# jyoung3131/oncilla

Measured on AMD Instinct MI355X. Metric: remote put/get GiB/s + p50 ocm_alloc latency, 4 KiB-1 GiB, 1/2/4/8 MI355X, higher is better.
Workload: dtype uint8

## Files before the change

### csrc/src/kernels/xfer.hip

```cpp
#include <hip/hip_runtime.h>

#include <cstring>

#include "ocm/xfer.h"
#include "xfer_copy.h"
#include "xfer_host.h"

namespace ocm {

namespace {

constexpr int kWaveSlice = (1 << kTileShift) / kWaves;
constexpr int kChunksPerWave = kWaveSlice / 1024;

template <class Cfg, bool MASKED = false>
__device__ __forceinline__ void copy_tiles(const XferArgs &a, uint32_t ext_mask = 0) {
    const uint64_t first = xfer_first_tile(a.rem_off, a.tile_shift);
    const uint64_t ntiles = xfer_tile_count(a.rem_off, a.len, a.tile_shift);
    const uint64_t r0 = a.rem_off;
    for (uint64_t ti = blockIdx.x; ti < ntiles; ti += gridDim.x) {
        if (MASKED && a.n_ext > 1) {
            const uint64_t lo = first + (ti << a.tile_shift);
            const uint64_t ts = lo > r0 ? lo : r0;
            const uint32_t e = (uint32_t)(ts >> a.unit_shift) % a.n_ext;
            if (!((ext_mask >> e) & 1u)) continue;
        }
        TileSpan s = tile_span(a, ti, first);
        copy_span<Cfg>(s.dst, s.src, s.n);
    }
}

template <int ST>
__global__ __launch_bounds__(kThreads) void xfer_reg_kernel(XferArgs a, XferDone d) {
    copy_tiles<BlockCopy<ST>>(a);
    xfer_publish(d);
}

typedef __attribute__((address_space(3))) void lds_void;
typedef const __attribute__((address_space(1))) void glob_void;

__device__ __forceinline__ bool full_aligned(const TileSpan &s) {
    return s.n == (1ull << kTileShift) && (((uintptr_t)s.dst | (uintptr_t)s.src) & 15u) == 0;
}

__device__ __forceinline__ void stage_tile(const char *src, char *buf, int wave, int lane) {
    const char *g = src + (size_t)wave * kWaveSlice + (size_t)lane * 16;
    char *l = buf + (size_t)wave * kWaveSlice;
#pragma unroll
    for (int c = 0; c < kChunksPerWave; c++)
        __builtin_amdgcn_global_load_lds((glob_void *)(g + c * 1024), (lds_void *)(l + c * 1024), 16, 0, 0);
}

template <bool NT>
__device__ __forceinline__ void drain_tile(char *dst, const char *buf, int wave, int lane) {
    const char *l = buf + (size_t)wave * kWaveSlice + (size_t)lane * 16;
    char *g = dst + (size_t)wave * kWaveSlice + (size_t)lane * 16;
    u32x4 v[kChunksPerWave];
#pragma unroll
    for (int c = 0; c < kChunksPerWave; c++) v[c] = *reinterpret_cast<const u32x4 *>(l + c * 1024);
#pragma unroll
    for (int c = 0; c < kChunksPerWave; c++)
        store16<NT>(reinterpret_cast<u32x4 *>(g + c * 1024), v[c]);
}

template <bool NT>
__device__ __forceinline__ void lds_stream(const XferArgs &a, char *lds, int wave, int lane, uint64_t ti,
                                           uint64_t first, uint64_t ntiles) {
    TileSpan cur = tile_span(a, ti, first);
    bool cur_staged = full_aligned(cur);
    if (cur_staged) stage_tile(cur.src, lds, wave, lane);
    int slot = 0;
    for (;;) {
        const uint64_t nt = ti + gridDim.x;
        TileSpan nxt;
        bool nxt_staged = false;
        if (nt < ntiles) {
            nxt = tile_span(a, nt, first);
            nxt_staged = full_aligned(nxt);
            if (nxt_staged) stage_tile(nxt.src, lds + (slot ^ 1) * (1 << kTileShift), wave, lane);
        }
        if (cur_staged) {
            if (nxt_staged)
                asm volatile("s_waitcnt vmcnt(8)" ::: "memory");
            else
                asm volatile("s_waitcnt vmcnt(0)" ::: "memory");
            drain_tile<NT>(cur.dst, lds + slot * (1 << kTileShift), wave, lane);
        } else {
            copy_span<BlockCopy<NT ? ST_NT : ST_PLAIN>>(cur.dst, cur.src, cur.n);
        }
        if (nt >= ntiles) break;
        ti = nt;
        cur = nxt;
        cur_staged = nxt_staged;
        slot ^= 1;
    }
}

template <bool NT>
__global__ __launch_bounds__(kThreads) void xfer_lds_kernel(XferArgs a, XferDone d) {
    __shared__ __attribute__((aligned(16))) char lds[2 * (1 << kTileShift)];
    const int wave = threadIdx.x >> 6, lane = threadIdx.x & 63;
    const uint64_t first = xfer_first_tile(a.rem_off, a.tile_shift);
    const uint64_t ntiles = xfer_tile_count(a.rem_off, a.len, a.tile_shift);
    uint64_t ti = blockIdx.x;
    if (ti < ntiles) lds_stream<NT>(a, lds, wave, lane, ti, first, ntiles);
    xfer_publish(d);
}

constexpr int kPcieUnroll = 2;
constexpr uint32_t kPcieTileShift = 13;
constexpr unsigned kPcieBlocksDefault = 128;

template <int SA>
using PcieCopy = CopyCfg<kThreads, kPcieUnroll, BufferAccess<kAuxNT, SA>>;

template <int SA>
__global__ __launch_bounds__(kThreads) void xfer_pcie_kernel(XferArgs a, XferDone d) {
    copy_tiles<PcieCopy<SA>>(a);
    xfer_publish(d);
}

__global__ __launch_bounds__(kThreads) void xfer_push_kernel(XferArgs a, uint32_t mask) {
    copy_tiles<BlockCopy<ST_NT>, true>(a, mask);
}

}

XferTuning xfer_tuning_from_env() {
    XferTuning t;
    const char *v = std::getenv("OCM_XFER_VARIANT");
    if (v && (!std::strcmp(v, "lds") || !std::strcmp(v, "2"))) t.variant = XFER_LDS;
    if (v && (!std::strcmp(v, "reg") || !std::strcmp(v, "1"))) t.variant = XFER_REG;
    if (v && (!std::strcmp(v, "pcie") || !std::strcmp(v, "4"))) t.variant = XFER_PCIE;
    if (v && (!std::strcmp(v, "push") || !std::strcmp(v, "5"))) t.variant = XFER_PUSH;
    t.max_blocks = kernels::env_int("OCM_XFER_BLOCKS", 0);
    t.nontemporal = kernels::env_int("OCM_XFER_NT", 1) != 0;
    t.write_through = kernels::env_int("OCM_XFER_NT", 1) == 2;
    return t;
}

hipError_t xfer_normalize(XferArgs &a) {
    if (a.n_ext < 1 || a.n_ext > (uint32_t)kXferMaxExtents) return hipErrorInvalidValue;
    a.tile_shift = kTileShift;
    if (a.n_ext > 1) {
        if (a.unit_shift < 4) return hipErrorInvalidValue;
        if (a.unit_shift < kTileShift) a.tile_shift = a.unit_shift;
    }
    return hipSuccess;
}

hipError_t xfer_launch(const XferArgs &in, const XferTuning &t, hipStream_t stream, const XferDone *done) {
    if (in.len == 0) return hipSuccess;
    XferArgs a = in;
    if (xfer_normalize(a) != hipSuccess) return hipErrorInvalidValue;
    const uint64_t ntiles = xfer_tile_count(a.rem_off, a.len, a.tile_shift);
    int variant = t.variant;
    if (variant == XFER_AUTO) variant = XFER_REG;
    const XferDone d0 = done ? *done : XferDone{};
    if (variant == XFER_PCIE) {
        if (a.tile_shift > kPcieTileShift) a.tile_shift = kPcieTileShift;
        const uint64_t tiles = xfer_tile_count(a.rem_off, a.len, a.tile_shift);
        const uint64_t cap = t.max_blocks > 0 ? (uint64_t)t.max_blocks : (uint64_t)kPcieBlocksDefault;
        const unsigned g = (unsigned)(tiles < cap ? tiles : cap);
        if (a.put && t.nontemporal)
            hipLaunchKernelGGL(xfer_pcie_kernel<kAuxSC1>, dim3(g), dim3(kThreads), 0, stream, a, d0);
        else
            hipLaunchKernelGGL(xfer_pcie_kernel<0>, dim3(g), dim3(kThreads), 0, stream, a, d0);
        return hipGetLastError();
    }
    if (a.tile_shift != kTileShift) variant = XFER_REG;
    int cap = t.max_blocks > 0 ? t.max_blocks : kernels::num_cus() * (variant == XFER_LDS ? 4 : 2);
    const unsigned grid = (unsigned)(ntiles < (uint64_t)cap ? ntiles : (uint64_t)cap);
    if (variant == XFER_LDS) {
        if (t.nontemporal)
            hipLaunchKernelGGL(xfer_lds_kernel<true>, dim3(grid), dim3(kThreads), 0, stream, a, d0);
        else
            hipLaunchKernelGGL(xfer_lds_kernel<false>, dim3(grid), dim3(kThreads), 0, stream, a, d0);
    } else {
        if (t.write_through)
            hipLaunchKernelGGL(xfer_reg_kernel<ST_WT>, dim3(grid), dim3(kThreads), 0, stream, a, d0);
        else if (t.nontemporal)
            hipLaunchKernelGGL(xfer_reg_kernel<ST_NT>, dim3(grid), dim3(kThreads), 0, stream, a, d0);
        else
            hipLaunchKernelGGL(xfer_reg_kernel<ST_PLAIN>, dim3(grid), dim3(kThreads), 0, stream, a, d0);
    }
    return hipGetLastError();
}

hipError_t xfer_push_launch(const XferArgs &in, uint32_t ext_mask, int max_blocks, hipStream_t stream) {
    if (in.len == 0 || ext_mask == 0) return hipSuccess;
    XferArgs a = in;
    if (a.put || xfer_normalize(a) != hipSuccess) return hipErrorInvalidValue;
    const uint64_t tiles = xfer_tile_count(a.rem_off, a.len, a.tile_shift);
    const uint32_t mine = (uint32_t)__builtin_popcount(ext_mask & ((1u << a.n_ext) - 1));
    const uint64_t own = a.n_ext > 1 ? (tiles * mine + a.n_ext - 1) / a.n_ext : tiles;
    const uint64_t cap = max_blocks > 0 ? (uint64_t)max_blocks : (uint64_t)kernels::num_cus() * 2;
    const unsigned g = (unsigned)(own < cap ? (own ? own : 1) : cap);
    hipLaunchKernelGGL(xfer_push_kernel, dim3(g), dim3(kThreads), 0, stream, a, ext_mask);
    return hipGetLastError();
}

hipError_t xfer_copy(void *dst, const void *src, uint64_t bytes, const XferTuning &t, hipStream_t stream) {
    XferArgs a;
    std::memset(&a, 0, sizeof(a));
    a.lin = const_cast<char *>(static_cast<const char *>(src));
    a.ext[0] = static_cast<char *>(dst);
    a.rem_off = 0;
    a.len = bytes;
    a.n_ext = 1;
    a.put = 1;
    return xfer_launch(a, t, stream);
}

}
```

### csrc/src/kernels/xfer_copy.h

```cpp
#pragma once
#include <hip/hip_runtime.h>

#include "ocm/list.h"
#include "ocm/xfer.h"

namespace ocm {

namespace {

typedef unsigned int u32x4 __attribute__((ext_vector_type(4)));

constexpr int kThreads = 256;
constexpr int kUnroll = 8;
constexpr uint32_t kTileShift = 15;
constexpr int kWaves = kThreads / 64;
static_assert(kWaves == kListWaves, "the host plans lists for workgroups of kListWaves waves");

enum StoreKind : int { ST_PLAIN = 0, ST_NT = 1, ST_WT = 2 };

__device__ __forceinline__ __amdgpu_buffer_rsrc_t span_rsrc(const void *base, uint32_t bytes) {
    const uint64_t b = reinterpret_cast<uint64_t>(base);
    const uint32_t lo = __builtin_amdgcn_readfirstlane((uint32_t)b);
    const uint32_t hi = __builtin_amdgcn_readfirstlane((uint32_t)(b >> 32));
    const uint32_t n = __builtin_amdgcn_readfirstlane(bytes);
    return __builtin_amdgcn_make_buffer_rsrc(reinterpret_cast<void *>(((uint64_t)hi << 32) | lo), 0, (int)n, 0x00020000);
}

constexpr int kAuxNT = 2, kAuxSC1 = 16;

template <int ST>
constexpr int store_aux() {
    return ST == ST_WT ? kAuxSC1 : ST == ST_NT ? kAuxNT : 0;
}
template <int ST>
constexpr int load_aux() {
    return ST == ST_WT ? kAuxSC1 : kAuxNT;
}

template <bool ATOMIC>
__device__ __forceinline__ void copy_byte(char *d, const char *s) {
    if constexpr (ATOMIC)
        __hip_atomic_store(d, __hip_atomic_load(s, __ATOMIC_RELAXED, __HIP_MEMORY_SCOPE_AGENT), __ATOMIC_RELAXED,
                           __HIP_MEMORY_SCOPE_AGENT);
    else
        *d = *s;
}

__device__ __forceinline__ uint64_t span_head(const char *dst, uint64_t n) {
    const uint64_t head = (16u - ((uintptr_t)dst & 15u)) & 15u;
    return head < n ? head : n;
}

template <bool NT>
__device__ __forceinline__ void store16(u32x4 *p, u32x4 v) {
    if constexpr (NT)
        __builtin_nontemporal_store(v, p);
    else
        *p = v;
}

template <int LA, int SA>
struct BufferAccess {
    static constexpr bool kRangeChecked = true;
    using Index = uint32_t;
    __amdgpu_buffer_rsrc_t rs, rd;
    __device__ __forceinline__ BufferAccess(char *dst, const char *src, uint32_t bytes)
        : rs(span_rsrc(src, bytes)), rd(span_rsrc(dst, bytes)) {}
    __device__ __forceinline__ u32x4 load(Index i) const {
        return __builtin_amdgcn_raw_buffer_load_b128(rs, (int)(i << 4), 0, LA);
    }
    __device__ __forceinline__ void store(Index i, u32x4 v) const {
        __builtin_amdgcn_raw_buffer_store_b128(v, rd, (int)(i << 4), 0, SA);
    }
};

template <bool NT>
struct PointerAccess {
    static constexpr bool kRangeChecked = false;
    using Index = uint64_t;
    const u32x4 *s;
    u32x4 *d;
    __device__ __forceinline__ PointerAccess(char *dst, const char *src, uint64_t)
        : s(reinterpret_cast<const u32x4 *>(src)), d(reinterpret_cast<u32x4 *>(dst)) {}
    __device__ __forceinline__ u32x4 load(Index i) const { return __builtin_nontemporal_load(s + i); }
    __device__ __forceinline__ void store(Index i, u32x4 v) const { store16<NT>(d + i, v); }
};

template <int LANES, int UNROLL, class ACCESS, bool ATOMIC_BYTES = false>
struct CopyCfg {
    static_assert(LANES == kThreads || LANES == 64, "a workgroup or one wave");
    static constexpr int kLanes = LANES, kRound = LANES * UNROLL;
    static constexpr int kVecs = UNROLL;
    static constexpr bool kAtomicBytes = ATOMIC_BYTES;
    using Access = ACCESS;
    __device__ static __forceinline__ int lane() { return LANES == 64 ? (int)(threadIdx.x & 63) : (int)threadIdx.x; }
};

template <int ST>
using BlockCopy = CopyCfg<kThreads, kUnroll, BufferAccess<load_aux<ST>(), store_aux<ST>()>, ST == ST_WT>;

template <class Cfg>
__device__ __forceinline__ void load_round(const typename Cfg::Access &acc, typename Cfg::Access::Index i,
                                           u32x4 (&v)[Cfg::kVecs]) {
#pragma unroll
    for (int k = 0; k < Cfg::kVecs; k++) v[k] = acc.load(i + k * Cfg::kLanes);
}

template <class Cfg>
__device__ __forceinline__ void store_round(const typename Cfg::Access &acc, typename Cfg::Access::Index i,
                                            const u32x4 (&v)[Cfg::kVecs]) {
#pragma unroll
    for (int k = 0; k < Cfg::kVecs; k++) acc.store(i + k * Cfg::kLanes, v[k]);
}

template <class Cfg>
__device__ __forceinline__ void copy_span(char *__restrict__ dst, const char *__restrict__ src, uint64_t n) {
    using Access = typename Cfg::Access;
    using Index = typename Access::Index;
    constexpr bool AB = Cfg::kAtomicBytes;
    const int lane = Cfg::lane();
    const uint64_t head = span_head(dst, n);
    if ((uint64_t)lane < head) copy_byte<AB>(dst + lane, src + lane);
    dst += head;
    src += head;
    n -= head;
    if (((uintptr_t)src & 15u) == 0 && (!Access::kRangeChecked || n < (1ull << 31))) {
        const Index nv = (Index)(n >> 4);
        const Access acc(dst, src, nv << 4);
        if constexpr (Access::kRangeChecked) {
            for (Index base = 0; base < nv; base += Cfg::kRound) {
                u32x4 v[Cfg::kVecs];
                load_round<Cfg>(acc, base + lane, v);
                store_round<Cfg>(acc, base + lane, v);
            }
        } else {
            Index i = lane;
            for (; i + (Cfg::kRound - Cfg::kLanes) < nv; i += Cfg::kRound) {
                u32x4 v[Cfg::kVecs];
                load_round<Cfg>(acc, i, v);
                store_round<Cfg>(acc, i, v);
            }
            for (; i < nv; i += Cfg::kLanes) acc.store(i, acc.load(i));
        }
        const uint64_t done = (uint64_t)nv << 4, tail = n & 15u;
        if ((uint64_t)lane < tail) copy_byte<AB>(dst + done + lane, src + done + lane);
    } else {
        for (uint64_t i = lane; i < n; i += Cfg::kLanes) copy_byte<AB>(dst + i, src + i);
    }
}

struct TileSpan {
    char *dst;
    const char *src;
    uint64_t n;
};

template <class Cfg>
__device__ __forceinline__ void copy_span2(const TileSpan &a, const TileSpan &b) {
    using Access = typename Cfg::Access;
    static_assert(Access::kRangeChecked, "a partial round relies on the range check");
    constexpr bool AB = Cfg::kAtomicBytes;
    const bool vec = (((uintptr_t)a.src ^ (uintptr_t)a.dst) & 15u) == 0 &&
                     (((uintptr_t)b.src ^ (uintptr_t)b.dst) & 15u) == 0 &&
                     a.n <= (uint64_t)Cfg::kRound * 16 && b.n <= (uint64_t)Cfg::kRound * 16;
    if (!vec) {
        copy_span<Cfg>(a.dst, a.src, a.n);
        copy_span<Cfg>(b.dst, b.src, b.n);
        return;
    }
    const int lane = Cfg::lane();
    const uint64_t ha = span_head(a.dst, a.n), hb = span_head(b.dst, b.n);
    if ((uint64_t)lane < ha) copy_byte<AB>(a.dst + lane, a.src + lane);
    if ((uint64_t)lane < hb) copy_byte<AB>(b.dst + lane, b.src + lane);
    const uint32_t nva = (uint32_t)((a.n - ha) >> 4), nvb = (uint32_t)((b.n - hb) >> 4);
    const Access acca(a.dst + ha, a.src + ha, nva << 4), accb(b.dst + hb, b.src + hb, nvb << 4);
    u32x4 va[Cfg::kVecs], vb[Cfg::kVecs];
    load_round<Cfg>(acca, lane, va);
    load_round<Cfg>(accb, lane, vb);
    store_round<Cfg>(acca, lane, va);
    store_round<Cfg>(accb, lane, vb);
    const uint64_t ta = (a.n - ha) & 15u, tb = (b.n - hb) & 15u;
    const uint64_t oa = ha + ((uint64_t)nva << 4), ob = hb + ((uint64_t)nvb << 4);
    if ((uint64_t)lane < ta) copy_byte<AB>(a.dst + oa + lane, a.src + oa + lane);
    if ((uint64_t)lane < tb) copy_byte<AB>(b.dst + ob + lane, b.src + ob + lane);
}

template <class E>
__device__ __forceinline__ char *stripe_ptr(const E &x, uint32_t n_ext, uint32_t unit_shift, uint64_t off) {
    if (n_ext == 1) return x.ext[0] + off;
    const uint64_t unit_mask = (1ull << unit_shift) - 1;
    const uint32_t u = (uint32_t)(off >> unit_shift);
    const uint32_t e = u % n_ext;
    const uint64_t eoff = ((uint64_t)(u / n_ext) << unit_shift) | (off & unit_mask);
    return x.ext[e] + eoff;
}

template <class E>
__device__ __forceinline__ TileSpan tile_span_of(const E &x, uint32_t n_ext, uint32_t unit_shift, uint32_t tile_shift,
                                                 char *lin, uint64_t rem_off, uint64_t len, uint32_t put, uint64_t ti,
                                                 uint64_t first_tile) {
    const uint64_t tile = 1ull << tile_shift;
    const uint64_t r0 = rem_off, r1 = rem_off + len;
    const uint64_t lo = first_tile + (ti << tile_shift);
    const uint64_t ts = lo > r0 ? lo : r0;
    const uint64_t te = (lo + tile) < r1 ? (lo + tile) : r1;
    char *rp = stripe_ptr(x, n_ext, unit_shift, ts);
    char *lp = lin + (ts - r0);
    TileSpan s;
    s.dst = put ? rp : lp;
    s.src = put ? lp : rp;
    s.n = te - ts;
    return s;
}

__device__ __forceinline__ TileSpan tile_span(const XferArgs &a, uint64_t ti, uint64_t first_tile) {
    return tile_span_of(a, a.n_ext, a.unit_shift, a.tile_shift, a.lin, a.rem_off, a.len, a.put, ti, first_tile);
}

__device__ __forceinline__ uint32_t uniform32(uint32_t v) { return __builtin_amdgcn_readfirstlane(v); }
__device__ __forceinline__ uint64_t uniform64(uint64_t v) {
    return ((uint64_t)uniform32((uint32_t)(v >> 32)) << 32) | uniform32((uint32_t)v);
}

template <class Args, class Op>
__device__ __forceinline__ uint32_t list_wave_start(const Args &a, uint32_t w, const Op **ops) {
    const bool inl = a.n_ops <= (uint32_t)(sizeof(Args::inline_ops) / sizeof(Op));
    *ops = inl ? a.inline_ops : a.ops;
    return inl ? 0u : a.wave_op[w];
}

__device__ __forceinline__ void block_release_system() {
    asm volatile("s_waitcnt vmcnt(0)" ::: "memory");
    __syncthreads();
    if (threadIdx.x == 0) __threadfence_system();
}

__device__ __forceinline__ void xfer_publish(const XferDone &d) {
    if (!d.flag) return;
    block_release_system();
    if (threadIdx.x == 0) {
        const unsigned old = __hip_atomic_fetch_add(d.cnt, 1u, __ATOMIC_ACQ_REL, __HIP_MEMORY_SCOPE_AGENT);
        if (old == gridDim.x - 1) {
            __hip_atomic_store(d.cnt, 0u, __ATOMIC_RELAXED, __HIP_MEMORY_SCOPE_AGENT);
            __hip_atomic_store(d.flag, d.val, __ATOMIC_RELEASE, __HIP_MEMORY_SCOPE_SYSTEM);
        }
    }
}

}

}
```

### csrc/src/lib/transfer.cpp

```cpp
#include "internal.h"

namespace ocmlib {



void segments(const lib_alloc *a, uint64_t rem_off, uint64_t len, std::vector<Seg> &out) {
    out.clear();
    const int n = (int)a->ext.size();
    if (n == 1 || a->stripe_unit == 0) {
        out.push_back({0, rem_off, 0, len});
        return;
    }
    const uint64_t unit = a->stripe_unit;
    uint64_t pos = rem_off, done = 0;
    while (done < len) {
        const uint64_t u = pos / unit, within = pos % unit;
        const uint64_t take = std::min(unit - within, len - done);
        out.push_back({(int)(u % n), (u / n) * unit + within, done, take});
        pos += take;
        done += take;
    }
}


int wait_event(hipEvent_t ev) {
    State &s = S();
    hipError_t e = hipSuccess;
    if (s.cfg.sync_mode == 1) {
        while ((e = hipEventQuery(ev)) == hipErrorNotReady) {
        }
    } else {
        e = hipEventSynchronize(ev);
    }
    if (e != hipSuccess) OCM_FAIL(-1, "event wait: %s", hipGetErrorString(e));
    return 0;
}

int honor_dep(lib_alloc *a, hipStream_t st, bool host_wait) {
    if (!a->dep_pending) return 0;
    a->dep_pending = false;
    hipError_t e = host_wait ? hipEventSynchronize(a->dep_ev) : hipStreamWaitEvent(st, a->dep_ev, 0);
    if (e != hipSuccess) OCM_FAIL(-1, "stream dependency: %s", hipGetErrorString(e));
    return 0;
}

int wait_alloc(lib_alloc *a) {
    State &s = S();
    if (!a || !a->async_pending) return 0;
    a->async_pending = false;
    if (!a->ev) return 0;
    DeviceGuard g(s.device);
    return wait_event(a->ev);
}

hipStream_t lane_stream(lib_alloc *a) {
    State &s = S();
    if (a->lane < 0) {
        if (s.lanes.empty()) {
            DeviceGuard g(s.device);
            for (int i = 0; i < std::max(1, s.cfg.n_lanes); i++) {
                hipStream_t st = nullptr;
                if (hipStreamCreateWithFlags(&st, hipStreamNonBlocking) != hipSuccess) {
                    (void)hipGetLastError();
                    break;
                }
                s.lanes.push_back(st);
            }
        }
        if (s.lanes.empty()) return s.stream;
        if (!s.lane_flags && s.cfg.launch_flags) {
            DeviceGuard g(s.device);
            const size_t nl = s.lanes.size();
            if (hipHostMalloc(reinterpret_cast<void **>(&s.lane_flags), nl * 128,
                              hipHostMallocCoherent | hipHostMallocMapped) != hipSuccess ||
                hipMalloc(reinterpret_cast<void **>(&s.lane_cnt), nl * 128) != hipSuccess ||
                hipMemset(s.lane_cnt, 0, nl * 128) != hipSuccess) {
                (void)hipGetLastError();
                s.cfg.launch_flags = false;
            } else {
                std::memset(s.lane_flags, 0, nl * 128);
                s.lane_flag_seq.assign(nl, 0);
            }
        }
        a->lane = s.next_lane++ % (int)s.lanes.size();
    }
    if (!a->ev) {
        DeviceGuard g(s.device);
        if (hipEventCreateWithFlags(&a->ev, hipEventDisableTiming) != hipSuccess) {
            (void)hipGetLastError();
            a->ev = nullptr;
            return s.stream;
        }
    }
    return s.lanes[a->lane];
}

int sync_stream() {
    State &s = S();
    if (!s.stream) return 0;
    DeviceGuard g(s.device);
    hipError_t e = hipSuccess;
    if (s.cfg.sync_mode == 0 || !s.done) {
        e = hipStreamSynchronize(s.stream);
    } else {
        e = hipEventRecord(s.done, s.stream);
        if (e == hipSuccess && s.cfg.sync_mode == 1) {
            while ((e = hipEventQuery(s.done)) == hipErrorNotReady) {
            }
        } else if (e == hipSuccess) {
            e = hipEventSynchronize(s.done);
        }
    }
    if (e != hipSuccess) OCM_FAIL(-1, "stream sync: %s", hipGetErrorString(e));
    return 0;
}

int async_done(lib_alloc *a, hipStream_t st) {
    State &s = S();
    if (st != s.stream && a->ev) {
        const hipError_t err = hipEventRecord(a->ev, st);
        if (err != hipSuccess) OCM_FAIL(-1, "event record failed: %s", hipGetErrorString(err));
    } else if (a->ev == nullptr && sync_stream() != 0) {
        return -1;
    }
    a->async_pending = a->ev != nullptr;
    return 0;
}

int wait_done(const XferDone &d, hipEvent_t ev) {
    for (unsigned spins = 1;; spins++) {
        if ((long long)(__atomic_load_n(d.flag, __ATOMIC_ACQUIRE) - d.val) >= 0) return 0;
        if ((spins & 4095) == 0) {
            const hipError_t e = hipEventQuery(ev);
            if (e == hipSuccess) return 0;
            if (e != hipErrorNotReady) OCM_FAIL(-1, "event wait: %s", hipGetErrorString(e));
        }
    }
}


static const XferTuning &dir_tuning(bool put) {
    State &s = S();
    const XferTuning &dt = s.dir_tuning[put ? 1 : 0];
    return dt.variant != XFER_AUTO ? dt : s.tuning;
}

static int pair_args(const lib_alloc *a, bool put, char *lin, uint64_t rem_off, uint64_t len, XferArgs *x) {
    std::memset(x, 0, sizeof(*x));
    x->lin = lin;
    x->rem_off = rem_off;
    x->len = len;
    x->put = put ? 1 : 0;
    if (pair_side(a, 0, x) < 0)
        OCM_FAIL(-1, "stripe unit %llu is not a power of two", (unsigned long long)a->stripe_unit);
    return 0;
}

static bool cpu_copies(Loc lloc, const Extent &e) {
    return S().device < 0 || (lloc != LOC_DEVICE && e.r.tier != TIER_GPU);
}

static hipError_t copy_segs(const lib_alloc *a, const Seg *segs, size_t n, bool put, char *lin, Loc lloc,
                            hipStream_t st) {
    for (const Seg *g = segs; g != segs + n; g++) {
        const Extent &e = a->ext[g->ext];
        const bool cpu = cpu_copies(lloc, e);
        char *r = (cpu ? e.hptr : e.dptr) + g->ext_off, *l = lin + g->lin_off;
        if (cpu) {
            std::memcpy(put ? r : l, put ? l : r, g->len);
            continue;
        }
        const hipError_t err = hipMemcpyAsync(put ? r : l, put ? l : r, g->len, hipMemcpyDefault, st);
        if (err != hipSuccess) return err;
    }
    return hipSuccess;
}


static int xfer_net(lib_alloc *a, bool put, char *lin, Loc lloc, uint64_t rem_off, uint64_t len) {
    State &s = S();
    std::vector<Seg> segs;
    segments(a, rem_off, len, segs);
    if (wait_alloc(a) != 0) return -1;
    if (honor_dep(a, nullptr, true) != 0) return -1;
    DeviceGuard dg(s.device);
    for (auto &g : segs) {
        const Extent &e = a->ext[g.ext];
        if (e.net) {
            if (net_piece(e, put, lin + g.lin_off, lloc, g.ext_off, g.len) != 0) return -1;
            continue;
        }
        if (copy_segs(a, &g, 1, put, lin, lloc, s.stream) != hipSuccess) OCM_FAIL(-1, "transfer launch failed");
        if (!cpu_copies(lloc, e) && sync_stream() != 0) return -1;
    }
    return 0;
}

static int xfer_cpu(lib_alloc *a, bool put, char *lin, Loc lloc, uint64_t rem_off, uint64_t len) {
    std::vector<Seg> segs;
    segments(a, rem_off, len, segs);
    (void)copy_segs(a, segs.data(), segs.size(), put, lin, lloc, nullptr);
    return 0;
}

static int xfer_service(lib_alloc *a, bool put, char *lin, uint64_t rem_off, uint64_t len) {
    State &s = S();
    XferArgs x;
    if (pair_args(a, put, lin, rem_off, len, &x) != 0) return -2;
    if (wait_alloc(a) != 0) return -2;
    if (honor_dep(a, nullptr, true) != 0) return -2;
    const unsigned solo = (!put && !a->any_gpu) ? std::min(s.cfg.svc_solo_tiles, s.cfg.svc_solo_tiles_host_get)
                                                : s.cfg.svc_solo_tiles;
    return service_xfer(x, solo, a->any_gpu, a->any_peer || s.cfg.svc_force_strict);
}

static int xfer_push(lib_alloc *a, char *lin, uint64_t rem_off, uint64_t len, hipStream_t st, bool async) {
    before_launch();
    if (push_get(a, lin, rem_off, len, st, async) != 0) return -1;
    return async ? async_done(a, st) : 0;
}

static int xfer_kernel(lib_alloc *a, bool put, char *lin, uint64_t rem_off, uint64_t len, hipStream_t st, bool async,
                       XferDone *done) {
    State &s = S();
    if ((s.cfg.svc_park_kernel || !a->any_gpu) && len > s.cfg.svc_limit(a)) service_park();
    before_launch();
    XferArgs x;
    if (pair_args(a, put, lin, rem_off, len, &x) != 0) return -1;
    XferTuning t = dir_tuning(put);
    if (t.variant == XFER_AUTO) {
        bool same_gpu = true;
        for (auto &e : a->ext) same_gpu &= e.r.tier == TIER_GPU && e.r.owner_gpu == s.device;
        t.variant = !a->any_gpu ? XFER_PCIE : (same_gpu && len <= (256ull << 20)) ? XFER_LDS : XFER_REG;
    }
    XferDone dn;
    if (done && async && len <= s.cfg.launch_flag_max && s.cfg.launch_flags && s.lane_flags && st != s.stream &&
        a->lane >= 0 && a->ev) {
        dn.flag = s.lane_flags + (size_t)a->lane * 16;
        dn.cnt = s.lane_cnt + (size_t)a->lane * 32;
        dn.val = ++s.lane_flag_seq[(size_t)a->lane];
    }
    const hipError_t err = xfer_launch(x, t, st, dn.flag ? &dn : nullptr);
    if (err != hipSuccess) OCM_FAIL(-1, "transfer launch failed: %s", hipGetErrorString(err));
    if (done) *done = dn;
    return async ? async_done(a, st) : sync_stream();
}

static int xfer_dma(lib_alloc *a, bool put, char *lin, Loc lloc, uint64_t rem_off, uint64_t len, hipStream_t st,
                    bool async) {
    service_park();
    std::vector<Seg> segs;
    segments(a, rem_off, len, segs);
    bool cpu_piece = false;
    for (auto &g : segs) cpu_piece |= cpu_copies(lloc, a->ext[g.ext]);
    hipError_t err = hipSuccess;
    if (cpu_piece && (err = hipStreamSynchronize(st)) != hipSuccess)
        OCM_FAIL(-1, "ordering a host copy after queued work: %s", hipGetErrorString(err));
    err = copy_segs(a, segs.data(), segs.size(), put, lin, lloc, st);
    if (err != hipSuccess) OCM_FAIL(-1, "transfer launch failed: %s", hipGetErrorString(err));
    return async ? async_done(a, st) : sync_stream();
}

int xfer(lib_alloc *a, bool put, char *lin, Loc lloc, uint64_t rem_off, uint64_t len, bool async, XferDone *done) {
    State &s = S();
    if (done) *done = XferDone{};
    if (len == 0) return 0;
    if (a->any_net) return xfer_net(a, put, lin, lloc, rem_off, len);
    if (s.device < 0) return xfer_cpu(a, put, lin, lloc, rem_off, len);
    DeviceGuard guard(s.device);
    const bool lin_dev = lloc == LOC_DEVICE;
    const bool dma_pick = dir_tuning(put).variant == XFER_DMA;
    if (lin_dev && a->all_dev_ok && !async && len <= s.cfg.svc_limit(a) && !dma_pick) {
        const int rc = xfer_service(a, put, lin, rem_off, len);
        if (rc == 0) return 0;
        if (rc == -2) return -1;
        OCM_WARN("copy service failed (%s); falling back to launches", last_error());
        s.cfg.svc_max = 0;
    }
    if (!async && wait_alloc(a) != 0) return -1;
    hipStream_t st = async ? lane_stream(a) : s.stream;
    if (honor_dep(a, st, false) != 0) return -1;
    const bool use_kernel =
        lin_dev && !dma_pick && (a->any_gpu || s.cfg.host_engine_kernel || len <= s.cfg.host_kernel_max);
    if (!use_kernel) return xfer_dma(a, put, lin, lloc, rem_off, len, st, async);
    if (!put && a->all_gpu && dir_tuning(false).variant == XFER_PUSH) return xfer_push(a, lin, rem_off, len, st, async);
    return xfer_kernel(a, put, lin, rem_off, len, st, async, done);
}


void push_release() {
    State &s = S();
    for (auto &kv : s.push) {
        DeviceGuard g(kv.first);
        if (kv.second.stream) (void)hipStreamSynchronize(kv.second.stream);
    }
}

static PushDev *push_dev(int d) {
    State &s = S();
    PushDev &p = s.push[d];
    if (p.ready) return &p;
    DeviceGuard g(d);
    if (d != s.device) {
        int can = 0;
        if (hipDeviceCanAccessPeer(&can, d, s.device) != hipSuccess || !can)
            OCM_FAIL(nullptr, "push get: GPU %d cannot reach GPU %d", d, s.device);
        const hipError_t pe = hipDeviceEnablePeerAccess(s.device, 0);
        if (pe != hipSuccess && pe != hipErrorPeerAccessAlreadyEnabled)
            OCM_FAIL(nullptr, "push get: peer access %d -> %d: %s", d, s.device, hipGetErrorString(pe));
        (void)hipGetLastError();
    }
    if (!p.stream && hipStreamCreateWithFlags(&p.stream, hipStreamNonBlocking) != hipSuccess)
        OCM_FAIL(nullptr, "push get: no stream on GPU %d", d);
    if (!p.done && hipEventCreateWithFlags(&p.done, hipEventDisableTiming) != hipSuccess)
        OCM_FAIL(nullptr, "push get: no event on GPU %d", d);
    p.ready = true;
    return &p;
}

int push_get(lib_alloc *a, char *lin, uint64_t rem_off, uint64_t len, hipStream_t st, bool async) {
    State &s = S();
    if (!a->all_gpu || a->any_net) OCM_FAIL(-1, "push get needs every extent in a GPU's HBM");
    std::map<int, uint32_t> owners;
    for (size_t i = 0; i < a->ext.size(); i++) {
        const int d = a->ext[i].r.owner_gpu;
        if (d < 0) OCM_FAIL(-1, "push get: extent %zu has no owner GPU", i);
        owners[d] |= 1u << i;
    }
    DeviceGuard g(s.device);
    if (!s.push_order && hipEventCreateWithFlags(&s.push_order, hipEventDisableTiming) != hipSuccess)
        OCM_FAIL(-1, "push get: no event");
    if (hipEventRecord(s.push_order, st) != hipSuccess) OCM_FAIL(-1, "push get: ordering event");
    std::vector<PushDev *> used;
    for (auto &kv : owners) {
        const int d = kv.first;
        PushDev *p = push_dev(d);
        if (!p) return -1;
        XferArgs x;
        if (pair_args(a, false, lin, rem_off, len, &x) != 0) return -1;
        for (size_t i = 0; i < a->ext.size(); i++) {
            x.ext[i] = nullptr;
            if (!((kv.second >> i) & 1u)) continue;
            x.ext[i] = extent_view(a->ext[i], d);
            if (!x.ext[i]) return -1;
        }
        DeviceGuard gd(d);
        hipError_t e = hipStreamWaitEvent(p->stream, s.push_order, 0);
        if (e == hipSuccess) e = xfer_push_launch(x, kv.second, s.dir_tuning[0].max_blocks, p->stream);
        if (e == hipSuccess) e = hipEventRecord(p->done, p->stream);
        if (e != hipSuccess) OCM_FAIL(-1, "push get on GPU %d: %s", d, hipGetErrorString(e));
        used.push_back(p);
        s.push_launches++;
    }
    for (PushDev *p : used) {
        const hipError_t e = async ? hipStreamWaitEvent(st, p->done, 0) : hipEventSynchronize(p->done);
        if (e != hipSuccess) OCM_FAIL(-1, "push get completion: %s", hipGetErrorString(e));
    }
    return 0;
}

int copy_local(void *dst, Loc dl, const void *src, Loc sl, size_t n) {
    State &s = S();
    if (n == 0) return 0;
    if (dl != LOC_DEVICE && sl != LOC_DEVICE) {
        std::memcpy(dst, src, n);
        return 0;
    }
    DeviceGuard g(s.device);
    hipError_t e;
    before_launch();
    if (dl == LOC_DEVICE && sl == LOC_DEVICE) {
        XferTuning t = s.tuning;
        if (t.variant == XFER_AUTO) t.variant = n <= (256ull << 20) ? XFER_LDS : XFER_REG;
        e = xfer_copy(dst, src, n, t, s.stream);
    } else
    {
        e = hipMemcpyAsync(dst, src, n, hipMemcpyDefault, s.stream);
    }
    if (e != hipSuccess) OCM_FAIL(-1, "local copy failed: %s", hipGetErrorString(e));
    return sync_stream();
}


}
```

Measured before the change: 52.84.

## Software-pipeline register copy kernel with buffer loads and route same-GPU traffic to it

Replaces the per-tile register copy with a double-buffered pipeline that issues the next tile's buffer loads before storing the current one, using explicit vmcnt waits so loads and stores overlap. For single-extent transfers under 2 GiB it builds one buffer resource and only advances an offset per tile, avoiding per-tile span computation. Misaligned head and tail tiles are handled separately by the first and last blocks. Auto selection no longer picks the LDS-staged kernel for same-GPU transfers and always uses the register path for GPU memory, which could be worse if the LDS path was better for local copies.

```diff
diff --git a/csrc/src/kernels/xfer.hip b/csrc/src/kernels/xfer.hip
--- a/csrc/src/kernels/xfer.hip
+++ b/csrc/src/kernels/xfer.hip
@@ -30,9 +30,103 @@
     }
 }
 
+__device__ __forceinline__ bool full_tiles_aligned(const XferArgs &a) {
+    uintptr_t m = (uintptr_t)a.lin - a.rem_off;
+#pragma unroll
+    for (uint32_t e = 0; e < (uint32_t)kXferMaxExtents; e++)
+        if (e < a.n_ext) m |= (uintptr_t)a.ext[e];
+    return (m & 15u) == 0;
+}
+
+template <bool FLAT>
+__device__ __forceinline__ TileRef full_tile_ref(const XferArgs &a, const TileRef &whole, uint64_t ti, uint64_t first) {
+    if constexpr (FLAT) {
+        TileRef t = whole;
+        t.off = (uint32_t)(first + (ti << kTileShift) - a.rem_off);
+        return t;
+    } else {
+        const TileSpan s = tile_span(a, ti, first);
+        return TileRef{span_rsrc(s.src, 1u << kTileShift), span_rsrc(s.dst, 1u << kTileShift), 0u};
+    }
+}
+
+template <int ST, bool FLAT>
+__device__ __forceinline__ void pipe_tiles(const XferArgs &a, uint64_t first, uint64_t t0, uint64_t t1) {
+    static_assert(3 * kUnroll < 64, "the waits below count up to 2 * kUnroll operations");
+    const uint64_t grid = gridDim.x;
+    uint64_t ti = blockIdx.x;
+    if (ti < t0) ti += grid;
+    if (ti >= t1) return;
+    const int voff = (int)threadIdx.x * 16;
+    TileRef whole{};
+    if constexpr (FLAT) {
+        const char *rem = a.ext[0] + a.rem_off;
+        whole.rs = span_rsrc(a.put ? a.lin : rem, (uint32_t)a.len);
+        whole.rd = span_rsrc(a.put ? rem : a.lin, (uint32_t)a.len);
+    }
+    u32x4 va[kUnroll], vb[kUnroll];
+    TileRef ra = full_tile_ref<FLAT>(a, whole, ti, first), rb;
+    tile_load<ST>(ra, voff, va);
+    if ((ti += grid) >= t1) {
+        vm_retire_to<0>();
+        tile_store<ST>(ra, voff, va);
+        return;
+    }
+    rb = full_tile_ref<FLAT>(a, whole, ti, first);
+    tile_load<ST>(rb, voff, vb);
+    vm_retire_to<kUnroll>();
+    tile_store<ST>(ra, voff, va);
+    for (;;) {
+        if ((ti += grid) >= t1) {
+            vm_retire_to<kUnroll>();
+            tile_store<ST>(rb, voff, vb);
+            return;
+        }
+        ra = full_tile_ref<FLAT>(a, whole, ti, first);
+        tile_load<ST>(ra, voff, va);
+        vm_retire_to<2 * kUnroll>();
+        tile_store<ST>(rb, voff, vb);
+        if ((ti += grid) >= t1) {
+            vm_retire_to<kUnroll>();
+            tile_store<ST>(ra, voff, va);
+            return;
+        }
+        rb = full_tile_ref<FLAT>(a, whole, ti, first);
+        tile_load<ST>(rb, voff, vb);
+        vm_retire_to<2 * kUnroll>();
+        tile_store<ST>(ra, voff, va);
+    }
+}
+
+template <int ST>
+__device__ __forceinline__ void copy_tiles_pipelined(const XferArgs &a) {
+    using Cfg = BlockCopy<ST>;
+    if (a.tile_shift != kTileShift || !full_tiles_aligned(a)) {
+        copy_tiles<Cfg>(a);
+        return;
+    }
+    const uint64_t first = xfer_first_tile(a.rem_off, kTileShift);
+    const uint64_t ntiles = xfer_tile_count(a.rem_off, a.len, kTileShift);
+    const uint64_t tile_mask = (1ull << kTileShift) - 1;
+    const uint64_t t0 = (a.rem_off & tile_mask) ? 1 : 0;
+    const uint64_t t1 = ntiles - (((a.rem_off + a.len) & tile_mask) ? 1 : 0);
+    if (t0 && blockIdx.x == 0) {
+        const TileSpan s = tile_span(a, 0, first);
+        copy_span<Cfg>(s.dst, s.src, s.n);
+    }
+    if (t1 < ntiles && t1 >= t0 && blockIdx.x == gridDim.x - 1) {
+        const TileSpan s = tile_span(a, ntiles - 1, first);
+        copy_span<Cfg>(s.dst, s.src, s.n);
+    }
+    if (a.n_ext == 1 && a.len < (1ull << 31))
+        pipe_tiles<ST, true>(a, first, t0, t1);
+    else
+        pipe_tiles<ST, false>(a, first, t0, t1);
+}
+
 template <int ST>
 __global__ __launch_bounds__(kThreads) void xfer_reg_kernel(XferArgs a, XferDone d) {
-    copy_tiles<BlockCopy<ST>>(a);
+    copy_tiles_pipelined<ST>(a);
     xfer_publish(d);
 }
 
diff --git a/csrc/src/kernels/xfer_copy.h b/csrc/src/kernels/xfer_copy.h
--- a/csrc/src/kernels/xfer_copy.h
+++ b/csrc/src/kernels/xfer_copy.h
@@ -217,6 +217,31 @@
     return tile_span_of(a, a.n_ext, a.unit_shift, a.tile_shift, a.lin, a.rem_off, a.len, a.put, ti, first_tile);
 }
 
+struct TileRef {
+    __amdgpu_buffer_rsrc_t rs, rd;
+    uint32_t off;
+};
+
+template <int ST>
+__device__ __forceinline__ void tile_load(const TileRef &t, int voff, u32x4 (&v)[kUnroll]) {
+#pragma unroll
+    for (int k = 0; k < kUnroll; k++)
+        v[k] = __builtin_amdgcn_raw_buffer_load_b128(t.rs, voff, (int)(t.off + k * kThreads * 16), load_aux<ST>());
+}
+
+template <int ST>
+__device__ __forceinline__ void tile_store(const TileRef &t, int voff, const u32x4 (&v)[kUnroll]) {
+#pragma unroll
+    for (int k = 0; k < kUnroll; k++)
+        __builtin_amdgcn_raw_buffer_store_b128(v[k], t.rd, voff, (int)(t.off + k * kThreads * 16), store_aux<ST>());
+}
+
+template <int N>
+__device__ __forceinline__ void vm_retire_to() {
+    static_assert(N >= 0 && N < 64, "vmcnt is a 6-bit counter");
+    asm volatile("s_waitcnt vmcnt(%0)" ::"n"(N) : "memory");
+}
+
 __device__ __forceinline__ uint32_t uniform32(uint32_t v) { return __builtin_amdgcn_readfirstlane(v); }
 __device__ __forceinline__ uint64_t uniform64(uint64_t v) {
     return ((uint64_t)uniform32((uint32_t)(v >> 32)) << 32) | uniform32((uint32_t)v);
diff --git a/csrc/src/lib/transfer.cpp b/csrc/src/lib/transfer.cpp
--- a/csrc/src/lib/transfer.cpp
+++ b/csrc/src/lib/transfer.cpp
@@ -229,9 +229,7 @@
     if (pair_args(a, put, lin, rem_off, len, &x) != 0) return -1;
     XferTuning t = dir_tuning(put);
     if (t.variant == XFER_AUTO) {
-        bool same_gpu = true;
-        for (auto &e : a->ext) same_gpu &= e.r.tier == TIER_GPU && e.r.owner_gpu == s.device;
-        t.variant = !a->any_gpu ? XFER_PCIE : (same_gpu && len <= (256ull << 20)) ? XFER_LDS : XFER_REG;
+        t.variant = !a->any_gpu ? XFER_PCIE : XFER_REG;
     }
     XferDone dn;
     if (done && async && len <= s.cfg.launch_flag_max && s.cfg.launch_flags && s.lane_flags && st != s.stream &&
```

New measurement: 52.74. Within noise of the previous version (-0.2%).
